# jj1bdx/airspy-fmradion

Hardware: AMD Instinct MI355X
Metric: IQ MS/s (FM stereo, 10 MS/s in), whole job (higher is better)
Workload: dtype f32 front end (stage A as a two-term fp16 split on the matrix cores, fp32 accumulate) / f64 after the discriminator

## Files before the change

### airspy-fmradion_amd/csrc/fmradion_amd.hip

```cpp
#include <hip/hip_runtime.h>
#include <hip/hip_ext.h>
#include <chrono>
#include <functional>
#include <thread>

#include <cstdarg>
#include <cstdio>
#include <algorithm>
#include <cstdlib>
#include <cstring>
#include <string>
#include <type_traits>
#include <vector>

#include "../../include/fmradion_amd.h"
#include "design.hpp"
#include "kernels.hpp"
#include "kernels_par.hpp"
#include "kernels_fused.hpp"
#include "kernels_decim16.hpp"
#include "kernels_chanbank.hpp"
#include "kernels_rds.hpp"
#include "kernels_spectrum.hpp"
#include "../host/fmradion_rds.hpp"

namespace {
#include "filter_tables.inc"

thread_local std::string g_err;

void set_err(const char *fmt, ...) {
  char buf[512];
  va_list ap;
  va_start(ap, fmt);
  vsnprintf(buf, sizeof buf, fmt, ap);
  va_end(ap);
  g_err = buf;
}

#define HIPCHK(expr)                                                                  \
  do {                                                                                \
    hipError_t e_ = (expr);                                                           \
    if (e_ != hipSuccess) {                                                           \
      set_err("%s failed: %s (%s:%d)", #expr, hipGetErrorString(e_), __FILE__, __LINE__); \
      return FMR_ERR_HIP;                                                             \
    }                                                                                 \
  } while (0)

constexpr double kFmRate = 384000.0;
constexpr double kPcmRate = 48000.0;
constexpr double kAmRate = 48000.0;
constexpr double kIfAtten = 140.0;
constexpr double kR8bAtten = 180.0, kR8bPassFrac = 0.98;
constexpr double kAudioAtten = 180.0;
constexpr int FMR_MODE_NONE = -1;
constexpr int C_AGC = 256, C_DC = 64, C_DE = 256, C_AM = 256, C_AM_DE = 128, K_AF_ITERS = 6;
#ifndef FMR_C_PLL_MIN
#define FMR_C_PLL_MIN 32
#endif
constexpr int C_PLL_MIN = FMR_C_PLL_MIN;
constexpr long long kSmallCall = 8192;
constexpr int kCPllSmall = 16;
constexpr unsigned kAgcWaitTicks = 50000000u;
constexpr int K_AGC_ITERS = 6, K_PLL_ITERS = 4;

template <class T>
struct DevBuf {
  T *p = nullptr;
  size_t n = 0;
  int alloc(size_t count) {
    n = count ? count : 1;
    HIPCHK(hipMalloc((void **)&p, n * sizeof(T)));
    HIPCHK(hipMemset(p, 0, n * sizeof(T)));
    return FMR_OK;
  }
  void release() { if (p) (void)hipFree(p); p = nullptr; }
};

struct KernelTime { const char *name; hipEvent_t a, b; };

}

using namespace fmr;

struct EnvKnobs {
  bool serial = false;
  int pipeline = -1;
#ifdef FMR_AB_PARTNERS
  int test_agc_late = 0;
#endif
  int fe_cus = 0;
  bool debug_taps = false;
  bool host_prof = false;
  bool no_fused = false;
#ifdef FMR_AB_PARTNERS
  bool pll_v1 = false;
#else
  static constexpr bool pll_v1 = false;
  static constexpr int test_agc_late = 0;
#endif
  double pll_rtol = -1.0;
  bool fe_stamps = false;
  bool evt_markers = false;
#ifdef FMR_DIAG_KNOBS
  int x_spare_aside = -1;
  int x_cpll = 0;
  int x_ballast = 0;
  int x_amtol = 0;
  int x_sumw = -1;
#else
  static constexpr int x_spare_aside = -1, x_cpll = 0, x_ballast = 0, x_sumw = -1, x_amtol = 0;
#endif
  static bool on(const char *n) { const char *e = getenv(n); return e && e[0] == '1'; }
  static bool set(const char *n) { return getenv(n) != nullptr; }
  void load() {
    serial = on("FMR_SERIAL"); debug_taps = on("FMR_DEBUG_TAPS");
    auto num = [](const char *n, int dflt) { const char *e = getenv(n); return (e && e[0]) ? atoi(e) : dflt; };
    pipeline = num("FMR_PIPELINE", -1); fe_cus = num("FMR_FE_CUS", 0);
    host_prof = on("FMR_HOST_PROF"); no_fused = on("FMR_NO_FUSED");
    fe_stamps = on("FMR_FE_STAMPS"); evt_markers = on("FMR_EVT_MARKERS");
#ifdef FMR_AB_PARTNERS
    test_agc_late = num("FMR_TEST_AGC_LATE", 0); pll_v1 = set("FMR_PLL_V1");
#endif
    if (const char *e = getenv("FMR_PLL_RTOL")) if (e[0]) pll_rtol = atof(e);
#ifdef FMR_DIAG_KNOBS
    x_spare_aside = num("FMR_X_SPARE_ASIDE", -1); x_cpll = num("FMR_X_CPLL", 0); x_ballast = num("FMR_X_BALLAST", 0); x_sumw = num("FMR_X_SUMW", -1); x_amtol = num("FMR_X_AMTOL", 0);
#endif
  }
};

struct fmr_chain {
  EnvKnobs env;
  fmr_config cfg{};
  int S = 1, mode = FMR_MODE_FM;
  bool has_rs = false, has_dec = true, fir_enable = false, stereo = false, pilot_shift = false;
  bool enable_mpf = false;
  hipStream_t stream = nullptr;
  bool dec_valid = true;
  bool if_valid = true;
  bool gain_valid = true;
  bool debug_taps = false;
  DeScan de_scan{};
  DevBuf<double> d_de_pow;
  double pll_rtol = 16.0;
  DevBuf<double> d_pll_wgr, d_pll_pre;
  DevBuf<PllSync> d_pll_sync;
  DevBuf<unsigned int> d_pll_tick2;
  int pll_jac_rounds = 1;
  double hp_fe = 0, hp_tab = 0, hp_dec = 0; long long hp_calls = 0; bool host_prof = false;
  hipStream_t tail = nullptr;
  bool pipelined = false;
  static constexpr int kPipe = 4;
  unsigned long long pipe_seq = 0;
  int ring_prev = -1;
  long long ring_prev_n = 0;
  DevBuf<float2> d_if_pp[kPipe];
  DevBuf<double> d_base_pp[kPipe], d_raw_pp[kPipe];
  DevBuf<FusedPart> d_part_pp[kPipe];
  DevBuf<int> d_stereo_pp[kPipe];
  float2 *if_slot(int q) { return q ? d_if_pp[q].p : d_if.p; }
  fm_mpx_t *base_slot(int q) { return reinterpret_cast<fm_mpx_t *>(q ? d_base_pp[q].p : d_base.p); }
  double *raw_slot(int q) { return q ? d_raw_pp[q].p : d_raw.p; }
  FusedPart *part_slot(int q) { return q ? d_part_pp[q].p : d_fused_part.p; }
  int *stereo_slot(int q) { return q ? d_stereo_pp[q].p : d_stereo_blk.p; }
  float2 *last_if = nullptr;
  hipEvent_t ev_fe[kPipe] = {};
  bool disc_commit_on_side = false;
  int sync_all() {
    if (int rc = flush_tail(nullptr)) return rc;
    for (hipStream_t st : {stream, side, side2, tail})
      if (st) HIPCHK(hipStreamSynchronize(st));
    return FMR_OK;
  }
  hipStream_t side = nullptr, side2 = nullptr;
  hipEvent_t ev_pll1 = nullptr;
  hipEvent_t ev_disc = nullptr, ev_pll = nullptr, ev_stats = nullptr, ev_fin = nullptr, ev_if = nullptr, ev_agc = nullptr,
             ev_tab = nullptr, ev_mono = nullptr;
  int pll_tick2_per_stream = 0;
  bool ev_agc_live = false;
  ResamplerDesign rs, ars;
  ResamplerCounter rsc, arsc;
  unsigned long long abs_in = 0;
  unsigned wait_multipath_blocks = 100;
  size_t max_in = 0, max_mid = 0, max_if = 0, max_amid = 0, max_au = 0;
  int max_blocks = 0;
  int H_in = 0, H_mid = 0, H_if = 0, H_a = 0, H_am = 0, H_pc = 0;
  int ntaps = 0, n_pilotcut = 0, mpf_N = 0, mpf_ref = 0;
  float h_coeff0 = 0.f;
  DevBuf<float2> d_in, d_in_halo, d_mid, d_if, d_fir, d_mpf, d_mpf_coeff, d_mpf_state;
  DevBuf<unsigned long long> d_agc_progress;
  std::vector<unsigned> agc_timeouts_seen;
  bool agc_beside_mpf = false;
  DevBuf<int> d_bphi, d_boff;
  int poly2_tile = 0;
  double nbfm_freq_dev = 8000.0;
  bool ssb_like = false;
  DevBuf<float2> d_ft_pre, d_ft_post;
  unsigned ft_index = 0;
  double af_ref = 0.6, af_rate = 0.001;
  int in_fmt = 0, in_bps = 8;
  enum class StageA : unsigned char { none, pass, bank, fused, decim16, decim2_16, decim2_24, decim };
  enum class StageB : unsigned char { none, fused, poly5h_disc, poly5h, poly4_am, poly4, poly3, poly2, poly_frac, poly };
  enum class IfForm : unsigned char { none, poly4_disc, block3_disc, block3, poly4_finish, block2, block };
  enum class FusedFe : unsigned char { none, if_only, disc };
  struct FeForms {
    StageB b = StageB::poly;
    FusedFe fused = FusedFe::none;
    bool decim16 = false;
    bool poly5h_disc = false;
    IfForm fir = IfForm::none;
  } fe;
  DevBuf<float> d_afrag_fir_fm;
  DevBuf<float> d_afrag_fir;
  int poly4_am_tile = 0;
  int poly5h_nkb = 0;
  float poly5h_inv_scale = 1.f;
  size_t poly5h_lds = 0;
  DevBuf<_Float16> d_afrag5h;
  DevBuf<float> d_afrag;
  DevBuf<unsigned short> d_dec16_afrag;
  DevBuf<float> d_run_ph;
  DevBuf<float> d_hB_last;
  DevBuf<unsigned short> d_fused_afragA;
  DevBuf<unsigned short> d_fused_afragB;
  float fused_hB_inv_scale = 1.f;
  DevBuf<FusedPart> d_fused_part;
  DevBuf<float> d_fused_mid32;
  DevBuf<float> d_zero16;
  DevBuf<unsigned long long> d_fe_stamps;
  int fe_stamps_n = 0;
  hipEvent_t ext_a = nullptr, ext_b = nullptr;
  int n_cu = 256;
  DevBuf<float> d_hBp;
  DevBuf<float> d_hpA;
  int qa = 0;
  unsigned fe_forms_a = 0, fe_forms_b = 0;
  bool bank = false;
  std::vector<int32_t> cb_off;
  unsigned long long cb_F = 0;
  DevBuf<float2> d_cb_taps;
  DevBuf<ChanPhase> d_cb_ph;
  unsigned cb_forms = 0;
  bool rds = false;
  static constexpr int kRdsSlots = 8;
  int rds_R = 0, rds_maxw = 0;
  size_t rds_slot_stride = 0;
  DevBuf<float> d_rds_h1, d_rds_h2, d_rds_xhalo;
  DevBuf<float2> d_rds_lo, d_rds_y1, d_rds_y2;
  DevBuf<RdsState> d_rds_state;
  DevBuf<RdsEst> d_rds_est;
  DevBuf<RdsRec> d_rds_rec;
  char *h_rds_slots = nullptr;
  unsigned long long *h_rds_mark = nullptr;
  long long rds_n = 0, rds_w = 0;
  unsigned long long rds_seq = 0, rds_drained = 0;
  unsigned long long rds_tap_seq = 0;
  double rds_gain = 1.0;
  std::vector<fmr_rds::Decoder> rds_dec;
  std::vector<RdsSlotHdr> rds_hdr;
  int rds_init();
  int rds_stage(const fm_mpx_t *base, long long N, hipStream_t st);
  void rds_drain();
  int in_rows() const { return bank ? 1 : S; }
  float2 *if_out = nullptr;
  long long if_out_stride = 0;
  int hB_pitch = 0;
  DevBuf<float> d_gain, d_dec, d_hA, d_hB, d_coeff, d_atan, d_if_rms_blk, d_bb_mean_blk, d_bb_rms_blk, d_blk_ph;
  DevBuf<double> d_base, d_raw, d_am0, d_am1, d_a10, d_a11, d_pc0, d_pc1, d_audio, d_ahA, d_ahB, d_pilotcut;
  DevBuf<int> d_tab, d_mpf_ok, d_stereo_blk;
  DevBuf<StreamState> d_state;
  bool serial_mode = false;
  int c_pll = 64;
  int H_b = 0;
  size_t max_ck = 0, max_agc_nc = 0, max_dc_nc = 0;
  DevBuf<double> d_pll_wfirst;
// ... 1824 lines not shown
  auto &d_iq = k.d_iq; auto &stride = k.stride; auto &nb = k.nb; auto &d_aud = k.d_aud; auto &astride = k.astride;
  auto &audio_len = k.audio_len; auto &N_in = k.N_in; auto &t_au_len = k.t_au_len; auto &N_if = k.N_if;
  auto &ifbuf = k.ifbuf; auto &N_au = k.N_au; auto &any_mpf = k.any_mpf;
  auto &amA_prev = k.amA_prev; auto &akB_prev = k.akB_prev; auto &an_prev = k.an_prev;
  auto &fused_n_tiles = k.fused_n_tiles; auto &fused_kb_ref = k.fused_kb_ref; auto &bt = k.bt;
  auto &if_stride = k.if_stride; auto &xin = k.xin; auto &x_stride = k.x_stride;
  auto &x_off = k.x_off; auto &disc_gain = k.disc_gain; auto &agc_on_side = k.agc_on_side;
  auto &agc_deferred = k.agc_deferred; auto &enqueue_agc = k.enqueue_agc;
  auto add_halo = [&](void *buf, long long stride_e, int H, long long N, int words = 2) { k.add_halo(buf, stride_e, H, N, words); };
  const CallPlan &p = k.plan;
  if (any_mpf) {
    timed("mpf", [&] {
      constexpr int NG4 = FMR_MPF_CH / 4 + 2;
      const int tpl4 = mpf_N <= 320 ? 5 : mpf_N <= 640 ? 10 : 20;
      const size_t lds4 = sizeof(float2) * ((size_t)mpf_N + FMR_MPF_CH + 8) + sizeof(float) * NG4 + sizeof(float2) * FMR_MPF_CH +
                          sizeof(double) * NG4 + sizeof(float2) * (tpl4 <= 10 ? 16 : 8) * 64 * (size_t)tpl4 + sizeof(int) * 16 +
                          sizeof(float2);
      auto go4 = [&](auto kern) {
        (void)hipFuncSetAttribute(reinterpret_cast<const void *>(kern), hipFuncAttributeMaxDynamicSharedMemorySize, (int)lds4);
        hipLaunchKernelGGL(kern, dim3(S), dim3(256), lds4, stream, xin, x_stride, x_off, d_gain.p, (long long)max_if,
                           bt, d_mpf.p, (long long)max_if, d_mpf_coeff.p, d_mpf_state.p, mpf_N, mpf_ref,
                           d_mpf_ok.p, d_state.p, agc_beside_mpf ? d_agc_progress.p : (const unsigned long long *)nullptr,
                           kAgcWaitTicks);
      };
      if (mpf_N <= 64 * 5) go4(k_mpf4<5>);
      else if (mpf_N <= 64 * 10) go4(k_mpf4<10>);
      else if (mpf_N <= 64 * 20) go4(k_mpf4<20>);
      else set_err("equaliser length out of range");
    });
  }
  if (agc_beside_mpf) {
    HIPCHK(hipStreamWaitEvent(stream, ev_agc, 0));
  }
  const long long base_stride = H_b + (long long)max_if;
  const long long de_stride = H_a + (long long)max_if;
  if (!p.b_disc && !p.fir_disc())
  timed("disc", [&] {
    hipLaunchKernelGGL((k_disc<256, fm_mpx_t>), dim3(nb, S), dim3(256), 0, stream, xin, x_stride, x_off, disc_gain,
                       (long long)max_if, any_mpf ? d_mpf.p : (float2 *)nullptr, (long long)max_if, d_mpf_ok.p, bt,
                       disc_nf, disc_bound, d_dec.p, (long long)max_if, k.base, base_stride, H_b,
                       d_bb_mean_blk.p, d_bb_rms_blk.p, d_state.p, p.fir == IfForm::none ? d_if_rms_blk.p : (float *)nullptr);
  });
  k.ev_mpx = (pipelined && p.b_disc) ? ev_fe[k.par] : ev_disc;
  if (k.ev_mpx == ev_disc) HIPCHK(hipEventRecord(ev_disc, stream));
  if (k.tail_deferred) { k.tail_deferred = false; if (int rc = flush_tail(ev_disc)) return rc; }
  HIPCHK(hipStreamWaitEvent(side, k.ev_mpx, 0));
  if (p.b == StageB::fused && !pipelined)
    timed_on(side, "in_halo", [&] {
      hipLaunchKernelGGL((k_update_in_halo<256, 0>), dim3(1, S), dim3(256), 0, side, d_in_halo.p, H_in, d_iq, (long long)stride, N_in);
    });
  const size_t stats_ballast = side_ballast();
  timed_on(side, "stats", [&] {
    hipLaunchKernelGGL(k_stats, dim3(S), dim3(FMR_STATS_THREADS), stats_ballast, side, bt, d_if_rms_blk.p, d_bb_mean_blk.p,
                       d_bb_rms_blk.p, d_state.p, S, (int)!(pipelined && p.b_disc),
                       (p.b_disc || p.fir_tail()) ? k.part : (const FusedPart *)nullptr, p.fir_tail() ? 8 * p.fir_runs.tiles : fused_n_tiles,
                       p.fir_tail() ? 0 : fused_kb_ref);
  });
  HIPCHK(hipEventRecord(ev_stats, side));
  disc_commit_on_side = !(pipelined && p.b_disc);
  bool fin_on_side = false, fin_covers_all = false;
  TailCtx t{};
  t.base = k.base; t.raw = k.raw; t.stereo_blk = k.stereo_blk; t.N_if = N_if; t.N_au = N_au; t.nb = nb; t.bt = bt;
  t.d_aud = d_aud; t.astride = (long long)astride; t.amA_prev = amA_prev; t.akB_prev = akB_prev;
  t.nch = stereo ? 2 : 1;
  for (int b = 0; b < nb; b++) t.au_max = std::max(t.au_max, t_au_len[b]);
  t.count_am = (int)(arsc.mA - amA_prev);
  if ((size_t)t.count_am > max_amid || (size_t)N_au > max_au) { set_err("internal audio capacity exceeded"); return FMR_ERR_CAPACITY; }
  t.a_top0 = (long long)ars.D * amA_prev + ars.ca() - an_prev;
  t.de_tout = std::min(4 * kDeBlock, ((kDeBlock * FMR_DE_LPL - FMR_DE_WARMUP - ars.NA - ars.D) / ars.D) & ~3);
  t.de_fused = !serial_mode && t.de_tout >= 64;
  t.dc_nc = (int)((N_au + C_DC - 1) / C_DC);
  t.dk.b0 = dcblock.b0; t.dk.b1 = dcblock.b1; t.dk.b2 = dcblock.b2; t.dk.a1 = dcblock.a1; t.dk.a2 = dcblock.a2;
  for (int j = 0; j < 4; j++) t.dk.ac[j] = dc_ac[j];
  for (int lv = 0; lv < 6; lv++) for (int j = 0; j < 4; j++) t.dk.agp[lv][j] = dc_agp[lv][j];
  const long long base_stride_ = base_stride;
  const long long am_stride = H_am + (long long)max_amid;
  const long long a1_stride = H_pc + (long long)max_au;
  t.can_split = stereo && !serial_mode && t.de_fused && (ars.LB == 3 && ars.MB == 8) && n_pilotcut <= FMR_PCUT_MAXTAPS;
  t.ev_mpx = k.ev_mpx;
  const bool split_mono = t.can_split && !pipelined;
  bool mono_enqueued = false;
  if (stereo) {
    auto tail_fn = [&](hipStream_t st, int ch_base, int nch_l) { tail_channels(t, st, ch_base, nch_l); };
    if (int rcp = run_fm_pll(k, base_stride_, split_mono, tail_fn, mono_enqueued, fin_on_side, fin_covers_all)) return rcp;
  }
  if (agc_deferred) { agc_deferred = false; if (int rca = enqueue_agc(nullptr)) return rca; }
  if (k.fe_post) { k.fe_post(); k.fe_post = nullptr; }
  t.fin_on_side = fin_on_side; t.fin_covers_all = fin_covers_all; t.agc_on_side = agc_on_side; t.mono_enqueued = mono_enqueued;

  if (!pipelined) {
    if (fir_enable) add_halo(ifbuf, if_stride, H_if, N_if);
    add_halo(k.base, base_stride, H_b, N_if, 1);
    if (stereo) add_halo(k.raw, base_stride, H_b, N_if);
  }
  if (!t.de_fused || debug_taps) {
    add_halo(d_base_de.p, de_stride, H_a, N_if);
    if (stereo) add_halo(d_raw_de.p, de_stride, H_a, N_if);
  }
  add_halo(d_am0.p, am_stride, H_am, t.count_am);
  if (stereo) add_halo(d_am1.p, am_stride, H_am, t.count_am);
  add_halo(d_a10.p, a1_stride, H_pc, N_au);
  if (stereo) add_halo(d_a11.p, a1_stride, H_pc, N_au);
  if (audio_len) for (int b = 0; b < nb; b++) audio_len[b] = (uint32_t)(stereo ? 2 * t_au_len[b] : t_au_len[b]);
  if (pipelined) {
    if (!stereo) HIPCHK(hipEventRecord(ev_pll, stream));
    t.ht = k.ht; k.ht.n = 0;
    t.seq = pipe_seq;
    tail_job = t;
    tail_pending = true;
    return FMR_OK;
  }
  return tail_stage(t, stream);
}

void fmr_chain::tail_channels(const TailCtx &t, hipStream_t st, int ch_base, int nch_l) {
  const long long base_stride = H_b + (long long)max_if, de_stride = H_a + (long long)max_if;
  const long long am_stride = H_am + (long long)max_amid, a1_stride = H_pc + (long long)max_au;
  const int count_am = t.count_am, de_tout = t.de_tout, dc_nc = t.dc_nc;
  const long long N_if = t.N_if, N_au = t.N_au, a_top0 = t.a_top0, amA_prev = t.amA_prev, akB_prev = t.akB_prev;
  const BlockTab &bt = t.bt;
  const int nb = t.nb;
  constexpr int DE_BLOCK = kDeBlock, DE_SLOTS = DE_BLOCK * FMR_DE_LPL;
  if (t.de_fused) {
    if (count_am > 0) {
      timed_on(st, "deemph_decim", [&] {
        const int tiles = (count_am + de_tout - 1) / de_tout;
        const size_t lds = sizeof(double) * (size_t)(DE_BLOCK * FMR_DE_RUN + 1);
        auto go = [&](auto kern) {
          hipLaunchKernelGGL(kern, dim3(tiles, S, nch_l), dim3(DE_BLOCK), lds, st, t.base, t.raw, base_stride, H_b,
                             (int)N_if, deemph.b0, deemph.a1, de_scan, 1, (int)(stereo && !pilot_shift), d_ahA.p,
                             ars.NA, ars.D, a_top0, count_am, de_tout, d_am0.p, d_am1.p, am_stride, H_am,
                             debug_taps ? d_base_de.p : (double *)nullptr,
                             debug_taps ? d_raw_de.p : (double *)nullptr, de_stride, H_a, ch_base);
        };
        if (ars.NA == 59 && ars.D == 3) go(k_deemph_decim<DE_BLOCK, 59, 3>);
        else go(k_deemph_decim<DE_BLOCK, 0, 0>);
      });
    }
  } else {
    timed_on(st, "deemph", [&] {
      const int nt = (int)((N_if + C_DE - 1) / C_DE);
      hipLaunchKernelGGL(k_deemph_par<C_DE>, dim3((nt + 63) / 64, S, nch_l), dim3(64), 0, st, t.base, t.raw,
                         base_stride, H_b, d_base_de.p, d_raw_de.p, de_stride, H_a, (int)N_if, deemph.b0, deemph.a1, 1,
                         (int)(stereo && !pilot_shift));
    });
    if (count_am > 0) {
      timed_on(st, "aud_decim", [&] {
        hipLaunchKernelGGL(k_aud_decim<128>, dim3((count_am + 127) / 128, S, nch_l), dim3(128), 0, st, d_base_de.p,
                           d_raw_de.p, de_stride, H_a, d_ahA.p, ars.NA, ars.D, a_top0, count_am, d_am0.p, d_am1.p,
                           am_stride, H_am);
      });
    }
  }
  if (N_au > 0) {
    timed_on(st, "aud_poly", [&] {
      if (ars.LB == 3 && ars.MB == 8) {
        constexpr int BLP = 256;
        const long long P_first = akB_prev / 3, P_last = (akB_prev + N_au - 1) / 3;
        const int tiles = (int)((P_last - P_first) / BLP + 1);
        const int lx = (BLP - 1) * (int)ars.MB + (int)((2 * ars.MB) / 3) + ars.TB;
        int ni_pad = (lx + (int)ars.MB - 1) / (int)ars.MB + 1;
        if ((ni_pad & 1) == 0) ni_pad++;
        hipLaunchKernelGGL((k_aud_poly2<BLP, 3, 8>), dim3(tiles, S, nch_l), dim3(BLP), sizeof(double) * (size_t)ars.MB * ni_pad,
                           st, d_am0.p, d_am1.p, am_stride, amA_prev - H_am, d_ahB.p, ars.TB,
                           akB_prev, (int)N_au, d_a10.p, d_a11.p, a1_stride, H_pc, ni_pad, H_am + count_am, ch_base);
      } else {
        hipLaunchKernelGGL(k_aud_poly<128>, dim3((unsigned)((N_au + 127) / 128), S, nch_l), dim3(128), 0, st,
                           d_am0.p, d_am1.p, am_stride, amA_prev - H_am, d_ahB.p, ars.TB, (unsigned)ars.LB,
                           (unsigned)ars.MB, (unsigned long long)akB_prev * ars.MB, (int)N_au, d_a10.p, d_a11.p,
                           a1_stride, H_pc);
      }
    });
    timed_on(st, "pilotcut", [&] {
      if (n_pilotcut <= FMR_PCUT_MAXTAPS && t.au_max <= 320)
        hipLaunchKernelGGL((k_pilotcut2<320, 320>), dim3(nb, S, nch_l), dim3(320), 0, st, d_a10.p, d_a11.p,
                           a1_stride, H_pc, bt, d_pilotcut.p, n_pilotcut, d_pc0.p, d_pc1.p, (long long)max_au, 1.0, ch_base);
      else if (n_pilotcut <= FMR_PCUT_MAXTAPS)
        hipLaunchKernelGGL((k_pilotcut2<320, 1280>), dim3(nb, S, nch_l), dim3(320), 0, st, d_a10.p, d_a11.p,
                           a1_stride, H_pc, bt, d_pilotcut.p, n_pilotcut, d_pc0.p, d_pc1.p, (long long)max_au, 1.0, ch_base);
      else
        hipLaunchKernelGGL(k_pilotcut<128>, dim3(nb, S, nch_l), dim3(128), 0, st, d_a10.p, d_a11.p, a1_stride, H_pc,
                           bt, d_pilotcut.p, n_pilotcut, d_pc0.p, d_pc1.p, (long long)max_au);
    });
  }
  if (N_au > 0 && !serial_mode)
    timed_on(st, "dc_pass1", [&] {
      hipLaunchKernelGGL(k_dc_pass1<C_DC>, dim3((dc_nc + 63) / 64, S, nch_l), dim3(64), 0, st, d_pc0.p, d_pc1.p,
                         (long long)max_au, (int)N_au, t.dk, d_dc_G.p, dc_nc, ch_base);
    });
}

int fmr_chain::tail_stage(const TailCtx &t, hipStream_t ts) {
  if (rds) if (int rc = rds_stage(t.base, t.N_if, ts)) return rc;
  const int nch = t.nch, dc_nc = t.dc_nc;
  const long long N_au = t.N_au;
  if (t.mono_enqueued) tail_channels(t, ts, 1, 1);
  else tail_channels(t, ts, 0, nch);
  if (t.mono_enqueued) HIPCHK(hipStreamWaitEvent(ts, ev_mono, 0));
  if (N_au > 0) {
    if (t.fin_on_side && serial_mode) HIPCHK(hipStreamWaitEvent(ts, ev_fin, 0));
    if (serial_mode) {
      timed_on(ts, "fm_out", [&] {
        hipLaunchKernelGGL(k_fm_out, dim3(S), dim3(64), 0, ts, d_pc0.p, d_pc1.p, (long long)max_au, t.bt, (int)N_au,
                           dcblock.b0, dcblock.b1, dcblock.b2, dcblock.a1, dcblock.a2, (int)stereo, (int)pilot_shift,
                           t.stereo_blk, t.d_aud, t.astride, d_state.p);
      });
    } else {
      timed_on(ts, "fm_out", [&] {
        const int dc_nw = std::max(1, std::min(FMR_DC_MAXW, (dc_nc + 64 * FMR_DC_K - 1) / (64 * FMR_DC_K)));
        hipLaunchKernelGGL(k_dc_nodes, dim3(S * nch), dim3(64 * dc_nw), 0, ts, d_dc_G.p, d_dc_start.p, dc_nc, t.dk,
                           d_state.p, S, nch);
        if (t.fin_on_side) (void)hipStreamWaitEvent(ts, ev_fin, 0);
        hipLaunchKernelGGL(k_dc_pass2_mux<C_DC>, dim3((dc_nc + 63) / 64, S), dim3(64), 0, ts, d_pc0.p, d_pc1.p,
                           (long long)max_au, t.bt, (int)N_au, t.dk, d_dc_start.p, dc_nc, (int)stereo, (int)pilot_shift,
                           t.stereo_blk, t.d_aud, t.astride, d_state.p);
      });
    }
  }
  if (!(t.fin_covers_all && N_au > 0)) {
    HIPCHK(hipStreamWaitEvent(ts, ev_stats, 0));
    if (t.agc_on_side) HIPCHK(hipStreamWaitEvent(ts, ev_agc, 0));
    if (t.fin_on_side) HIPCHK(hipStreamWaitEvent(ts, ev_fin, 0));
  }
  return FMR_OK;
}

static double rds_pulse(double t) {
  const double td = 1.0 / 1187.5, u = 8.0 * t / td;
  if (std::fabs(std::fabs(u) - 1.0) < 1e-9) return M_PI / 4.0;
  return std::cos(M_PI * u / 2.0) / (1.0 - u * u);
}
int fmr_chain::rds_init() {
  const size_t need = max_if / kRdsD + 5 * 1300 + 256;
  rds_R = 1;
  while ((size_t)rds_R < need) rds_R <<= 1;
  rds_maxw = (int)(((double)max_if * 19.0) / (double)(kRdsWin * kRdsSym)) + 3;
  std::vector<float> h1(kRdsNT1), h2(kRdsNT2);
  double sum = 0.0;
  std::vector<double> hd(kRdsNT1);
  for (int k = 0; k < kRdsNT1; k++) {
    const double x = k - (kRdsNT1 - 1) / 2.0, fc = 12000.0 / kFmRate;
    const double sinc = 2.0 * fc * (x == 0.0 ? 1.0 : std::sin(2.0 * M_PI * fc * x) / (2.0 * M_PI * fc * x));
    const double w = 0.42 - 0.5 * std::cos(2.0 * M_PI * k / (kRdsNT1 - 1)) + 0.08 * std::cos(4.0 * M_PI * k / (kRdsNT1 - 1));
    hd[k] = sinc * w;
    sum += hd[k];
  }
  for (int k = 0; k < kRdsNT1; k++) h1[k] = (float)(hd[k] / sum);
  const double fs2 = kFmRate / kRdsD, T = 0.5 / 1187.5;
  for (int j = 0; j < kRdsNT2; j++) h2[j] = (float)rds_pulse((j - (kRdsNT2 - 1) / 2) / fs2);
  auto d = [&](double t) { return rds_pulse(t) - rds_pulse(t - T); };
  double y0 = 0.0, yT = 0.0;
  for (int j = 0; j < kRdsNT2; j++) {
    const double u = (j - (kRdsNT2 - 1) / 2) / fs2;
    y0 += h2[j] * 0.5 * d(-u);
    yT += h2[j] * 0.5 * d(T - u);
  }
  rds_gain = std::fabs(y0 - yT);
  std::vector<float2> lo(128);
  for (int i = 0; i < 128; i++) lo[i] = make_float2((float)std::cos(2.0 * M_PI * i / 128.0), (float)-std::sin(2.0 * M_PI * i / 128.0));
  int rc;
  if ((rc = upload(d_rds_h1, h1.data(), h1.size()))) return rc;
  if ((rc = upload(d_rds_h2, h2.data(), h2.size()))) return rc;
  if ((rc = upload(d_rds_lo, lo.data(), lo.size()))) return rc;
  if ((rc = d_rds_xhalo.alloc((size_t)S * kRdsHalo))) return rc;
  if ((rc = d_rds_y1.alloc((size_t)S * rds_R))) return rc;
  if ((rc = d_rds_y2.alloc((size_t)S * rds_R))) return rc;
  if ((rc = d_rds_state.alloc((size_t)S))) return rc;
  if ((rc = d_rds_est.alloc((size_t)S * rds_maxw))) return rc;
  if ((rc = d_rds_rec.alloc((size_t)S * (rds_maxw + 1)))) return rc;
  rds_slot_stride = (rds_slot_bytes(rds_maxw) + 63) & ~(size_t)63;
  HIPCHK(hipHostMalloc((void **)&h_rds_slots, rds_slot_stride * (size_t)S * kRdsSlots, hipHostMallocCoherent));
  HIPCHK(hipHostMalloc((void **)&h_rds_mark, sizeof(unsigned long long), hipHostMallocCoherent));
  *h_rds_mark = 0;
  rds_dec.assign(S, fmr_rds::Decoder());
  rds_hdr.assign(S, RdsSlotHdr{});
  return FMR_OK;
}

int fmr_chain::rds_stage(const fm_mpx_t *base, long long N, hipStream_t st) {
  rds_tap_seq = 0;
  if (N <= 0) return FMR_OK;
  const long long base_stride = H_b + (long long)max_if;
  const long long n0 = rds_n, m0 = (n0 + kRdsD - 1) / kRdsD, m1 = (n0 + N + kRdsD - 1) / kRdsD;
  const int cnt = (int)(m1 - m0);
  timed_on(st, "rds_mix", [&] {
    if (cnt > 0) {
      hipLaunchKernelGGL(k_rds_mix<256>, dim3((cnt + 255) / 256, S), dim3(256), 0, st, base, base_stride, H_b, d_rds_xhalo.p,
                         n0, m0, cnt, d_rds_h1.p, d_rds_lo.p, d_rds_y1.p, rds_R);
      hipLaunchKernelGGL(k_rds_mf<256>, dim3((cnt + 255) / 256, S), dim3(256), 0, st, d_rds_y1.p, d_rds_y2.p, rds_R, m0, cnt,
                         d_rds_h2.p);
    }
    hipLaunchKernelGGL(k_rds_halo, dim3(S), dim3(kRdsHalo), 0, st, base, base_stride, H_b, d_rds_xhalo.p, n0, (int)N);
  });
  rds_n = n0 + N;
  auto ready = [&](long long w) {
    const double T = (double)((w + 1) * kRdsWin * kRdsSym + kRdsSym) / 19.0;
    return (long long)std::floor((T + kRdsDelay1) / kRdsD + kRdsDelay2) + 3 <= m1;
  };
  int nw = 0;
  while (nw < rds_maxw && ready(rds_w + nw)) nw++;
  if (nw == 0) { HIPCHK(hipGetLastError()); return FMR_OK; }
  const unsigned long long seq = ++rds_seq;
  if (seq > (unsigned long long)kRdsSlots) {
    if (int rc = wait_mark(h_rds_mark, seq - kRdsSlots)) return rc;
    rds_drain();
  }
  char *slot = h_rds_slots + (size_t)(seq % kRdsSlots) * S * rds_slot_stride;
  timed_on(st, "rds_sym", [&] {
    hipLaunchKernelGGL(k_rds_est, dim3(nw, S), dim3(64), 0, st, d_rds_y2.p, rds_R, rds_w, d_rds_est.p, rds_maxw);
    hipLaunchKernelGGL(k_rds_scan, dim3((S + 63) / 64), dim3(64), 0, st, d_rds_est.p, nw, rds_w, rds_maxw, d_rds_state.p,
                       d_rds_rec.p, slot, rds_slot_stride, S);
    hipLaunchKernelGGL(k_rds_bits, dim3(nw, S), dim3(128), 0, st, d_rds_y2.p, rds_R, d_rds_rec.p, rds_maxw, slot,
                       rds_slot_stride);
  });
  hipLaunchKernelGGL(k_signal_host, dim3(1), dim3(1), 0, st, h_rds_mark, seq);
  rds_w += nw;
  rds_tap_seq = seq;
  HIPCHK(hipGetLastError());
  return FMR_OK;
// ... 1124 lines not shown
```

Measured before the change: 282,500.

## Fuse audio polyphase resampler with pilot-cut FIR in one tail kernel

Adds a kernel that computes the 3/8 polyphase audio resampler output into LDS and then applies the pilot-cut FIR directly from shared memory, using an overlapping halo of HP outputs per tile. This replaces two launches and the global round trip of the intermediate audio buffer on the default path. The trade-offs are that some resampler outputs are recomputed at tile overlaps, the block is larger at 320 threads, and the pilot-cut is evaluated per output with a binary search over block offsets. The old two-kernel LB=3/MB=8 path now sits behind a compile-time flag.

```diff
diff --git a/airspy-fmradion_amd/csrc/fmradion_amd.hip b/airspy-fmradion_amd/csrc/fmradion_amd.hip
--- a/airspy-fmradion_amd/csrc/fmradion_amd.hip
+++ b/airspy-fmradion_amd/csrc/fmradion_amd.hip
@@ -17,6 +17,7 @@
 #include "design.hpp"
 #include "kernels.hpp"
 #include "kernels_par.hpp"
+#include "kernels_tail.hpp"
 #include "kernels_fused.hpp"
 #include "kernels_decim16.hpp"
 #include "kernels_chanbank.hpp"
@@ -95,9 +96,11 @@
   bool no_fused = false;
 #ifdef FMR_AB_PARTNERS
   bool pll_v1 = false;
+  bool x_tail_split = false;
 #else
   static constexpr bool pll_v1 = false;
   static constexpr int test_agc_late = 0;
+  static constexpr bool x_tail_split = false;
 #endif
   double pll_rtol = -1.0;
   bool fe_stamps = false;
@@ -120,7 +123,7 @@
     host_prof = on("FMR_HOST_PROF"); no_fused = on("FMR_NO_FUSED");
     fe_stamps = on("FMR_FE_STAMPS"); evt_markers = on("FMR_EVT_MARKERS");
 #ifdef FMR_AB_PARTNERS
-    test_agc_late = num("FMR_TEST_AGC_LATE", 0); pll_v1 = set("FMR_PLL_V1");
+    test_agc_late = num("FMR_TEST_AGC_LATE", 0); pll_v1 = set("FMR_PLL_V1"); x_tail_split = on("FMR_X_TAIL_SPLIT");
 #endif
     if (const char *e = getenv("FMR_PLL_RTOL")) if (e[0]) pll_rtol = atof(e);
 #ifdef FMR_DIAG_KNOBS
@@ -2251,8 +2254,25 @@
       });
     }
   }
+  const bool tail_fused = N_au > 0 && ars.LB == 3 && ars.MB == 8 && n_pilotcut <= FMR_PCUT_MAXTAPS && !env.x_tail_split;
+  if (tail_fused) {
+    timed_on(st, "aud_poly", [&] {
+      constexpr int BLP = 320;
+      const int np = BLP - (n_pilotcut - 1 + 2) / 3;
+      const long long P_first = akB_prev / 3, P_last = (akB_prev + N_au - 1) / 3;
+      const int tiles = (int)((P_last - P_first) / np + 1);
+      const int lx = (BLP - 1) * (int)ars.MB + (int)((2 * ars.MB) / 3) + ars.TB;
+      int ni_pad = (lx + (int)ars.MB - 1) / (int)ars.MB + 1;
+      if ((ni_pad & 1) == 0) ni_pad++;
+      hipLaunchKernelGGL((k_audB_pcut<BLP, 3, 8>), dim3(tiles, S, nch_l), dim3(BLP),
+                         sizeof(double) * ((size_t)ars.MB * ni_pad + FMR_PCUT_MAXTAPS), st, d_am0.p, d_am1.p, am_stride,
+                         amA_prev - H_am, d_ahB.p, ars.TB, akB_prev, (int)N_au, d_a10.p, d_a11.p, a1_stride, H_pc, ni_pad,
+                         H_am + count_am, bt, d_pilotcut.p, n_pilotcut, d_pc0.p, d_pc1.p, (long long)max_au, ch_base);
+    });
+  } else
   if (N_au > 0) {
     timed_on(st, "aud_poly", [&] {
+#ifdef FMR_AB_PARTNERS
       if (ars.LB == 3 && ars.MB == 8) {
         constexpr int BLP = 256;
         const long long P_first = akB_prev / 3, P_last = (akB_prev + N_au - 1) / 3;
@@ -2263,7 +2283,9 @@
         hipLaunchKernelGGL((k_aud_poly2<BLP, 3, 8>), dim3(tiles, S, nch_l), dim3(BLP), sizeof(double) * (size_t)ars.MB * ni_pad,
                            st, d_am0.p, d_am1.p, am_stride, amA_prev - H_am, d_ahB.p, ars.TB,
                            akB_prev, (int)N_au, d_a10.p, d_a11.p, a1_stride, H_pc, ni_pad, H_am + count_am, ch_base);
-      } else {
+      } else
+#endif
+      {
         hipLaunchKernelGGL(k_aud_poly<128>, dim3((unsigned)((N_au + 127) / 128), S, nch_l), dim3(128), 0, st,
                            d_am0.p, d_am1.p, am_stride, amA_prev - H_am, d_ahB.p, ars.TB, (unsigned)ars.LB,
                            (unsigned)ars.MB, (unsigned long long)akB_prev * ars.MB, (int)N_au, d_a10.p, d_a11.p,
diff --git a/airspy-fmradion_amd/csrc/kernels_tail.hpp b/airspy-fmradion_amd/csrc/kernels_tail.hpp
--- /dev/null
+++ b/airspy-fmradion_amd/csrc/kernels_tail.hpp
@@ -0,0 +1,113 @@
+#pragma once
+#include "kernels.hpp"
+
+namespace fmr {
+
+template <int BLOCK, int LBT, int MB>
+__global__ __launch_bounds__(BLOCK) void k_audB_pcut(
+    const double *__restrict__ m0, const double *__restrict__ m1, long long m_stride, long long mid_abs0,
+    const double *__restrict__ hB, int TB, long long k0, int count,
+    double *__restrict__ a0, double *__restrict__ a1, long long a_stride, int a_halo, int ni_pad, int mid_valid,
+    BlockTab bt, const double *__restrict__ coeff, int ntaps,
+    double *__restrict__ p0, double *__restrict__ p1, long long p_stride, int ch_base) {
+  extern __shared__ __attribute__((aligned(16))) double lds_tp[];
+  const int s = blockIdx.y, ch = blockIdx.z + ch_base;
+  const int tid = threadIdx.x;
+  const double *mid = (ch ? m1 : m0) + (long long)s * m_stride;
+  double *hist = (ch ? a1 : a0) + (long long)s * a_stride + a_halo;
+  double *y = (ch ? p1 : p0) + (long long)s * p_stride;
+  const int order = ntaps - 1, half_order = (order - 1) / 2;
+  const int HP = (order + LBT - 1) / LBT;
+  const int NP = BLOCK - HP;
+  double *cs = lds_tp + MB * ni_pad;
+  for (int j = tid; j < ntaps; j += BLOCK) cs[j] = coeff[j];
+  const int W = TB >> 1;
+  const long long Pt = k0 / LBT + (long long)blockIdx.x * NP - HP;
+  const long long a0i = Pt * MB - W + 1;
+  int off[LBT], phi[LBT];
+#pragma unroll
+  for (int p = 0; p < LBT; p++) { off[p] = (p * MB) / LBT; phi[p] = (p * MB) % LBT; }
+  const int lx = (BLOCK - 1) * MB + off[LBT - 1] + TB;
+  for (int e0 = 0; e0 < lx; e0 += 8 * BLOCK) {
+    double v[8];
+#pragma unroll
+    for (int t = 0; t < 8; t++) {
+      const int e = e0 + t * BLOCK + tid;
+      const long long idx = a0i + e - mid_abs0;
+      v[t] = (e < lx && idx >= 0 && idx < mid_valid) ? mid[idx] : 0.0;
+    }
+#pragma unroll
+    for (int t = 0; t < 8; t++) {
+      const int e = e0 + t * BLOCK + tid;
+      if (e < lx) lds_tp[(e % MB) * ni_pad + e / MB] = v[t];
+    }
+  }
+  __syncthreads();
+  double acc[LBT];
+#pragma unroll
+  for (int p = 0; p < LBT; p++) acc[p] = 0.0;
+  int j = 0;
+  for (; j + 8 <= TB; j += 8) {
+    double hv[LBT][8], xv[LBT][8];
+#pragma unroll
+    for (int p = 0; p < LBT; p++)
+#pragma unroll
+      for (int u = 0; u < 8; u++) {
+        const int jj = off[p] + j + u;
+        hv[p][u] = hB[(size_t)phi[p] * TB + j + u];
+        xv[p][u] = lds_tp[(jj % MB) * ni_pad + tid + jj / MB];
+      }
+#pragma unroll
+    for (int u = 0; u < 8; u++)
+#pragma unroll
+      for (int p = 0; p < LBT; p++) acc[p] += hv[p][u] * xv[p][u];
+  }
+  for (; j < TB; j++) {
+#pragma unroll
+    for (int p = 0; p < LBT; p++) {
+      const int jj = off[p] + j;
+      acc[p] += hB[(size_t)phi[p] * TB + j] * lds_tp[(jj % MB) * ni_pad + tid + jj / MB];
+    }
+  }
+  const long long kb = Pt * LBT - k0;
+  __syncthreads();
+#pragma unroll
+  for (int p = 0; p < LBT; p++) {
+    const long long k = kb + (long long)tid * LBT + p;
+    double v = acc[p];
+    if (k < 0) v = (k >= -(long long)a_halo) ? hist[k] : 0.0;
+    else if (k < count && k >= (long long)count - a_halo && tid >= HP) hist[k] = v;
+    lds_tp[tid * LBT + p] = v;
+  }
+  __syncthreads();
+  const double *xs = lds_tp;
+  auto block_of = [&](long long k, int lo, int hi) {
+    while (lo < hi) {
+      const int md = (lo + hi + 1) >> 1;
+      if (bt.au_off[md] <= (int)k) lo = md; else hi = md - 1;
+    }
+    return lo;
+  };
+  const long long k_first = max(kb + HP * LBT, 0ll), k_last = min(kb + (long long)BLOCK * LBT, (long long)count) - 1;
+  if (k_last < k_first) return;
+  const int b_first = block_of(k_first, 0, bt.nb - 1), b_last = block_of(k_last, b_first, bt.nb - 1);
+  for (int r = HP * LBT + tid; r < BLOCK * LBT; r += BLOCK) {
+    const long long k = kb + r;
+    if (k < 0 || k >= count) continue;
+    const int lo = block_of(k, b_first, b_last);
+    const int i = (int)k - bt.au_off[lo];
+    const double *xc = xs + r;
+    double a = 0.0;
+    if (i < order) {
+      for (int q = i + 1; q <= order; q++) a += xc[-q] * cs[q];
+      for (int q = 1; q <= i; q++) a += xc[-q] * cs[q];
+    } else {
+#pragma unroll 8
+      for (int q = 0; q <= half_order; q++) a += (xc[-q] + xc[-(order - q)]) * coeff[q];
+      if ((order % 2) == 0) a += xc[-(order / 2)] * coeff[order / 2];
+    }
+    y[k] = a;
+  }
+}
+
+}
```

Result: slower. 265,700 (-6.0%).
